# HENDRIX-ZT2/pyaudiorestoration

Measured on AMD Instinct MI355X. Metric: Msamples/sec resampled (192 kHz varispeed), higher is better.
Workload: dtype f32 near taps, far taps (|n| >= 3) as float16 hi + lo x 2^-12 filter banks on v_mfma_f32_16x16x32_f16 with f32 accumulation / f64 positions

## Files before the change

### pyaudiorestoration_amd/csrc/pos.hip

```cpp
#include "par_common.h"
#include "pos_plan.h"
#include <math.h>
#include <vector>

#pragma clang fp contract(off)

namespace par {

struct AddU128 {
  using T = U128;
  __device__ static T identity() { return T{0ull, 0ull}; }
  __device__ static T combine(T a, T b) {
    T r;
    r.lo = a.lo + b.lo;
    r.hi = a.hi + b.hi + (r.lo < a.lo ? 1ull : 0ull);
    return r;
  }
};
struct AddF64 {
  using T = double;
  __device__ static T identity() { return 0.0; }
  __device__ static T combine(T a, T b) { return a + b; }
};
struct ComposeP {
// ... 778 lines not shown
    double rr[kCk];
    const double a0 = (double)k;
#pragma unroll
    for (int u = 0; u < kCk; ++u) rr[u] = ramp_recip(a0 + (double)u, r);
#pragma unroll
    for (int u = 0; u < kCk; ++u) x = x + rr[u];
    if (k + kCk < c.n) ck[c.slot0 + k / kCk + 1] = x;
  }
  for (; k < c.k1; ++k) x = x + ramp_recip((double)k, r);
  if (__double_as_longlong(x) != __double_as_longlong(x_end)) atomicOr(&h->flags, kFlagVerify);
  if (c.j == c.J - 1) S[c.i] = x;
}

__global__ void k_inject_verify_fault(PlanHeader* __restrict__ h) { atomicOr(&h->flags, kFlagVerify); }

__global__ void k_publish_ck(PlanHeader* __restrict__ h, int64_t ck_len) {
  h->ck_len = ck_len;
  h->ck_valid = (h->flags & ~kFlagCapAmbiguous) ? 0 : 1;
  h->flags &= ~kFlagCkOverflow;
}

__device__ __forceinline__ SegFast seg_fast_record(const double* __restrict__ sp, const double* __restrict__ seg_off, long long x,
                                                   long long n) {
  const double s0 = sp[x], s1 = sp[x + 1], off = seg_off[x];
  SegFast f;
  const bool off_ok = fabs(off) < 4.0e18;
  const double ro = off_ok ? rint(off) : 0.0;
  f.foff = off_ok ? off - ro : 0.0;
  f.A = (long long)ro;
  f.n = n < 0x7fffffffll ? (int)n : 0x7fffffff;
  f.step = n >= 2 ? (s1 - s0) / (double)(n - 1) : 0.0;
  const double smin = s0 < s1 ? s0 : s1, smax = s0 < s1 ? s1 : s0;
  const double st2 = f.step * f.step, sm2 = smin * smin;
  f.fast = off_ok && n >= 2 && n < 0x7fffffffll && smin >= 0.0625 && smax <= 64.0 && st2 * st2 <= 1.296e-13 * sm2 * sm2 * smin;
  if (f.fast && fabs(f.step) <= 5.0e-5 * smin) f.fast = fabs(f.step) <= 2.7e-6 * smin ? 3 : 2;
  return f;
}

__device__ __forceinline__ void tile_entry(const double* __restrict__ sp, const int64_t* __restrict__ seg_start,
                                           const double* __restrict__ seg_off, int64_t nseg, const double* __restrict__ ck,
                                           int64_t ck_len, int64_t* __restrict__ tile_seg, long long* __restrict__ tile_st,
                                           TileHdr* __restrict__ hdr, const long long x, const long long n_tiles,
                                           const long long sample, const long long lo, const bool lazy) {
  tile_seg[x] = lo;
  for (int q = 0; q < kTileStarts; ++q) tile_st[x * kTileStarts + q] = lo + q <= nseg ? seg_start[lo + q] : LLONG_MAX;
  if (x < n_tiles) {
    const long long start = seg_start[lo], k = sample - start, b = k >> 3;
    static_assert(kCk == 8, "k >> 3");
    const double off = seg_off[lo];
    const bool off_ok = fabs(off) < 4.0e18;
    const double ro = off_ok ? rint(off) : 0.0;
    const long long slot = ck_slot0(start, lo) + b;
    const double ckv = lazy ? (lazy_segment_ok(seg_start[lo + 1] - start, sp[lo], sp[lo + 1])
                                   ? lazy_prefix(sp[lo], (sp[lo + 1] - sp[lo]) / (double)(seg_start[lo + 1] - start - 1), (double)(k + 1))
                                   : 0.0)
                            : ((b && slot < ck_len) ? ck[slot] : 0.0);
    const double rel = (off_ok ? off - ro : 0.0) + ckv;
    const bool ok = off_ok && fabs(rel) < 1.0e15 && ro > -0x1p61 && ro < 0x1p61;
    TileHdr hd;
    hd.anchor = ok ? ((long long)ro + (long long)rint(rel)) & ~1ll : 0ll;
    hd.c_last = 0;
    hd.iT = lo;
    hd.mn_rel = 0;
    bool may_unity = false, may_slow = false;
    for (long long q = lo; q < nseg && seg_start[q] <= sample + kSincTileOutputs; ++q) {
      may_unity = may_unity || !(sp[q] < kUnityHintBelow) || !(sp[q + 1] < kUnityHintBelow);
      may_slow = may_slow || !(sp[q] >= kSlowHintBelow) || !(sp[q + 1] >= kSlowHintBelow);
    }
    hd.flags = (ok ? 0 : 1) | (may_unity ? kTileMayUnity : 0) | (may_slow ? kTileMaySlow : 0) | (lazy ? kTileLazy : 0);
    hdr[x] = hd;
  }
}

__device__ __forceinline__ void tile_seg_body(const double* __restrict__ sp, const int64_t* __restrict__ seg_start,
                           const double* __restrict__ seg_off, int64_t nseg, const double* __restrict__ ck, int64_t ck_len,
                           int64_t max_tiles, int64_t* __restrict__ tile_seg, SegFast* __restrict__ seg_fast,
                           long long* __restrict__ tile_st, TileHdr* __restrict__ hdr, PlanHeader* __restrict__ h, const int64_t x) {
  const long long len_out = h->len_out;
  const long long n_tiles = (len_out + kSincTileOutputs - 1) / kSincTileOutputs;
  if (n_tiles + 1 > max_tiles) {
    if (x == 0 && len_out > 0) atomicOr(&h->flags, kFlagCkOverflow);
    return;
  }
  if (x < nseg) {
    const long long a = seg_start[x], b = seg_start[x + 1];
    if (b > a && a < len_out && ck_slot0(a, x) + (b - a + kCk - 1) / kCk > ck_len)
      atomicOr(&h->flags, kFlagCkOverflow);
    seg_fast[x] = seg_fast_record(sp, seg_off, x, b - a);
  }
  if (x > n_tiles || len_out <= 0) return;
  const long long sample = x < n_tiles ? x * kSincTileOutputs : len_out - 1;
  long long lo = 0, hi = nseg;
  while (lo < hi) {
    const long long mid = (lo + hi + 1) >> 1;
    if (seg_start[mid] <= sample) lo = mid; else hi = mid - 1;
  }
  if (lo < nseg) tile_entry(sp, seg_start, seg_off, nseg, ck, ck_len, tile_seg, tile_st, hdr, x, n_tiles, sample, lo, false);
}

__global__ void k_tile_seg(const double* __restrict__ sp, const int64_t* __restrict__ seg_start,
                           const double* __restrict__ seg_off, int64_t nseg, const double* __restrict__ ck, int64_t ck_len,
                           int64_t max_tiles, int64_t* __restrict__ tile_seg, SegFast* __restrict__ seg_fast,
                           long long* __restrict__ tile_st, TileHdr* __restrict__ hdr, PlanHeader* __restrict__ h) {
  tile_seg_body(sp, seg_start, seg_off, nseg, ck, ck_len, max_tiles, tile_seg, seg_fast, tile_st, hdr, h,
                (int64_t)blockIdx.x * blockDim.x + threadIdx.x);
}

__global__ void k_tile_seg_publish(const double* __restrict__ sp, const int64_t* __restrict__ seg_start,
                                   const double* __restrict__ seg_off, int64_t nseg, const double* __restrict__ ck, int64_t ck_len,
                                   int64_t max_tiles, int64_t* __restrict__ tile_seg, SegFast* __restrict__ seg_fast,
                                   long long* __restrict__ tile_st, TileHdr* __restrict__ hdr, PlanHeader* __restrict__ h,
                                   int64_t n_items) {
  __shared__ int is_last;
  if (h->lazy_fail) return;
  for (int64_t x0 = (int64_t)blockIdx.x * blockDim.x; x0 < n_items; x0 += (int64_t)gridDim.x * blockDim.x)
    tile_seg_body(sp, seg_start, seg_off, nseg, ck, ck_len, max_tiles, tile_seg, seg_fast, tile_st, hdr, h, x0 + threadIdx.x);
  __threadfence();
  __syncthreads();
  if (threadIdx.x == 0) is_last = atomicAdd(&h->done_tile_seg_publish, 1) == (int)gridDim.x - 1;
  __syncthreads();
  if (!is_last || threadIdx.x != 0) return;
  __threadfence();
  h->done_tile_seg_publish = 0;
  const int fl = __hip_atomic_load(&h->flags, __ATOMIC_RELAXED, __HIP_MEMORY_SCOPE_AGENT);
  h->ck_len = ck_len;
  h->ck_valid = (fl & ~kFlagCapAmbiguous) ? 0 : 1;
  h->flags = fl & ~kFlagCkOverflow;
}

__global__ __launch_bounds__(256) void k_tile_seg_lazy(const double* __restrict__ sp, const int64_t* __restrict__ seg_start,
                                                       const double* __restrict__ seg_off, int64_t nseg,
                                                       int64_t* __restrict__ tile_seg, SegFast* __restrict__ seg_fast,
                                                       long long* __restrict__ tile_st, TileHdr* __restrict__ hdr,
                                                       const PlanHeader* __restrict__ h) {
  if (h->ck_valid != 2) return;
  const long long x = (long long)blockIdx.x * blockDim.x + threadIdx.x;
  if (x >= nseg) return;
  const long long len_out = h->len_out;
  const long long n_tiles = (len_out + kSincTileOutputs - 1) / kSincTileOutputs;
  const long long a = seg_start[x], b = seg_start[x + 1];
  seg_fast[x] = seg_fast_record(sp, seg_off, x, b - a);
  if (b <= a || a >= len_out) return;
  for (long long T = (a + kSincTileOutputs - 1) / kSincTileOutputs; T * kSincTileOutputs < b && T < n_tiles; ++T)
    tile_entry(sp, seg_start, seg_off, nseg, nullptr, 0, tile_seg, tile_st, hdr, T, n_tiles, T * kSincTileOutputs, x, true);
  if (len_out - 1 < b) tile_entry(sp, seg_start, seg_off, nseg, nullptr, 0, tile_seg, tile_st, hdr, n_tiles, n_tiles, len_out - 1, x, true);
}

struct BlockPoly {
  double a0;
  double a1m1;
  double a2;
};
__device__ __forceinline__ double recip_nr(double b) {
  double x = __builtin_amdgcn_rcp(b);
  x = __builtin_fma(x, __builtin_fma(-b, x, 1.0), x);
  return __builtin_fma(x, __builtin_fma(-b, x, 1.0), x);
}
__device__ __forceinline__ BlockPoly piece_poly(double base, double rc, double z, int d0) {
  const double rp = -(rc * z), cz = rc * z * z, dd0 = (double)d0;
  const double s2m = (dd0 - 1.0) * dd0 * (2.0 * dd0 - 1.0) * (1.0 / 6.0);
  BlockPoly q;
  q.a0 = ((base + rc * (1.0 - dd0)) + 0.5 * rp * (dd0 - dd0 * dd0)) - cz * s2m;
  q.a1m1 = ((rc - 1.0) + 0.5 * rp) + cz * (1.0 / 6.0);
  q.a2 = 0.5 * rp + 0.5 * cz;
  return q;
}
__device__ __forceinline__ BlockPoly block_poly(double foff, double step, double s0, double k, int uk, double ckv, bool fast) {
  const double rc = recip_nr(__builtin_fma(step, k + 16.0, s0));
  const double z = rc * step;
  double cprev = ckv;
  if (uk) {
    if (fast) {
      const double x = z * (-0.5 * (double)(uk + 1) - 16.0);
      const double r = rc * __builtin_fma(x, __builtin_fma(x, -x, x) - 1.0, 1.0);
      cprev += r * (double)uk * __builtin_fma(z * z, (double)(uk * uk - 1) * (1.0 / 12.0), 1.0);
    } else {
      for (int v = 0; v < uk; ++v) cprev += recip_nr(__builtin_fma(step, k - (double)(uk - v), s0));
    }
  }
  return piece_poly(foff + cprev, rc, z, -16);
}
__device__ __forceinline__ bool irel_ok(long long rel) { return rel > -32000 && rel < 32000; }

__global__ __launch_bounds__(256) void k_block_rec2(const double* __restrict__ sp, const int64_t* __restrict__ seg_start,
                                                    int64_t nseg, const SegFast* __restrict__ seg_fast,
                                                    const TileHdr* __restrict__ hdr, BlockRec* __restrict__ rec,
                                                    BlockRec2* __restrict__ rec2, const PlanHeader* __restrict__ h) {
  const long long i = (long long)blockIdx.x * blockDim.x + threadIdx.x;
  if (i < 1 || i >= nseg || !h->ck_valid) return;
  const long long start = seg_start[i];
  const int us = (int)(start & (kRec - 1));
  if (us == 0 || start >= h->len_out) return;
  const SegFast s1 = seg_fast[i];
  const double rc = recip_nr(__builtin_fma(s1.step, (double)(16 - us), sp[i]));
  const BlockPoly b1 = piece_poly(s1.foff, rc, rc * s1.step, us - 16);
  const double r1 = rint(b1.a0);
  const long long rel = s1.A + (long long)r1 - hdr[start / kSincTileOutputs].anchor;
  BlockRec2 o2;
  o2.w0 = (unsigned)((int)rel << 16);
  o2.F = (float)(b1.a0 - r1);
  o2.e1 = (float)b1.a1m1;
  o2.e2 = (float)b1.a2;
  rec2[start >> kRecShift] = o2;
  if (!(fabs(b1.a0) < 1.0e9 && irel_ok(rel))) atomicOr(&rec[start >> kRecShift].w0, kRecSlow1);
}

__global__ __launch_bounds__(256) void k_block_rec(const double* __restrict__ sp, const int64_t* __restrict__ seg_start,
                                                   int64_t nseg, const double* __restrict__ ck,
                                                   const int64_t* __restrict__ tile_seg, const long long* __restrict__ tile_st,
                                                   const SegFast* __restrict__ seg_fast, const TileHdr* __restrict__ hdr,
                                                   BlockRec* __restrict__ rec, const PlanHeader* __restrict__ h) {
  const long long len_out = h->len_out;
  if (!h->ck_valid) return;
  const long long g = (long long)blockIdx.x * blockDim.x + threadIdx.x;
  const long long jb = g * kRec;
  if (jb >= len_out) return;
  const long long T = g / kBlocksPerTile;
  const long long j0 = T * kSincTileOutputs;
  const long long iT = tile_seg[T];
  int Sr[kTileStarts];
#pragma unroll
  for (int q = 0; q < kTileStarts; ++q) {
    const long long d = tile_st[T * kTileStarts + q] - j0;
    Sr[q] = d < -0x40000000ll ? -0x40000000 : (d > 0x40000000ll ? 0x40000000 : (int)d);
  }
  const int jr = (int)(jb - j0);
  int si = 0;
#pragma unroll
  for (int q = 1; q < kTileStarts; ++q) si += jr >= Sr[q];
  long long i = iT + si;
  long long k;
  double kd;
  int rem;
  long long slot0;
  if (si < kTileStarts - 1 && Sr[0] > -0x40000000) {
    int sr = Sr[0], nr = Sr[1];
#pragma unroll
    for (int q = 1; q < kTileStarts - 1; ++q) {
      if (si == q) {
        sr = Sr[q];
        nr = Sr[q + 1];
      }
    }
    k = jr - sr;
    kd = (double)(jr - sr);
    const int d = nr - jr;
    rem = d < kRec + 1 ? d : kRec + 1;
    slot0 = ck_slot0(j0 + sr, i);
  } else {
    long long hi = tile_seg[T + 1];
    while (i < hi) {
      const long long mid = (i + hi + 1) >> 1;
      if (seg_start[mid] <= jb) i = mid; else hi = mid - 1;
    }
    const long long start = seg_start[i], d = seg_start[i + 1] - jb;
    k = jb - start;
    kd = (double)k;
    rem = d < kRec + 1 ? (int)d : kRec + 1;
    slot0 = ck_slot0(start, i);
  }
  const long long i1 = i + 1 < nseg ? i + 1 : i;
  const SegFast sf = seg_fast[i];
  const SegFast s1 = seg_fast[i1];
  const double sp0 = sp[i], sp1 = sp[i1];
  const TileHdr hd = hdr[T];
  const long long b = k >> 3;
  const int uk = (int)(k & 7);
  static_assert(kCk == 8, "k >> 3");
  BlockPoly q0;
  if (hd.flags & kTileLazy) {
    const double rc = recip_nr(__builtin_fma(sf.step, kd + 16.0, sp0));
    q0 = piece_poly(sf.foff + lazy_prefix(sp0, sf.step, kd), rc, rc * sf.step, -16);
  } else {
    const double ckv = b ? ck[slot0 + b] : 0.0;
    q0 = block_poly(sf.foff, sf.step, sp0, kd, uk, ckv, sf.fast != 0);
  }
  const double r0 = rint(q0.a0);
  const long long rel0 = sf.A + (long long)(int)r0 - hd.anchor;
  const bool range0 = fabs(q0.a0) < 1.0e9 && sf.A > -(1ll << 61) && sf.A < (1ll << 61) && irel_ok(rel0) && !(hd.flags & 1);
  const unsigned ustar = rem < kRec ? (unsigned)rem : (unsigned)kRec;
  const long long ul = j0 + kSincTileOutputs >= len_out ? len_out - 1 - jb : -1;
  const unsigned slow0 = !(sf.fast >= 2 && range0 && fabs(q0.a1m1) <= 0.03125) || (ul >= 0 && ul < (long long)ustar);
  unsigned slow1 = 0u, end1 = 0u, cubic = sf.fast == 2;
  if (ustar < (unsigned)kRec) {
    const int need = kRec - (int)ustar;
    end1 = s1.n == need;
    slow1 = !(i + 1 < nseg && s1.fast >= 2 && s1.n >= need && s1.A > -(1ll << 61) && s1.A < (1ll << 61) && sp1 >= 0.971 &&
              sp1 <= 1.031) ||
            (ul >= (long long)ustar && ul < kRec);
    cubic |= s1.fast == 2;
  }
  BlockRec o;
  const bool e0 = (ustar < (unsigned)kRec) || rem == kRec;
  if (end1) slow1 = 1u;
  o.w0 = ((unsigned)((int)rel0 << 16)) | (ustar - 1u) | (e0 ? kRecE0 : 0u) | (end1 ? kRecE1 : 0u) | (slow0 ? kRecSlow0 : 0u) |
         (slow1 ? kRecSlow1 : 0u) | (cubic ? kRecCubic : 0u) | ((e0 ? ustar - 1u : 63u) << kRecLastShift);
  o.F = (float)(q0.a0 - r0);
  o.e1 = (float)q0.a1m1;
  o.e2 = (float)q0.a2;
  rec[g] = o;
}

constexpr int kRecLazySegs = 64;
#ifndef PAR_REC_EXP
#define PAR_REC_EXP 0
#endif
__device__ __forceinline__ double recip_nr_c(double b) {
#pragma clang fp contract(fast)
  double x = __builtin_amdgcn_rcp(b);
  x = x + x * (1.0 - b * x);
  return x + x * (1.0 - b * x);
}
__device__ __forceinline__ BlockPoly piece_poly_c(double base, double rc, double z, int d0) {
#pragma clang fp contract(fast)
  const double rp = -(rc * z), cz = rc * z * z, dd0 = (double)d0;
  const double s2m = (dd0 - 1.0) * dd0 * (2.0 * dd0 - 1.0) * (1.0 / 6.0);
  BlockPoly q;
  q.a0 = ((base + rc * (1.0 - dd0)) + 0.5 * rp * (dd0 - dd0 * dd0)) - cz * s2m;
  q.a1m1 = ((rc - 1.0) + 0.5 * rp) + cz * (1.0 / 6.0);
  q.a2 = 0.5 * rp + 0.5 * cz;
  return q;
}
__device__ __forceinline__ double lazy_prefix_nr(double s0, double step, double K) {
#pragma clang fp contract(fast)
  const double rc = recip_nr_c(__builtin_fma(step, 0.5 * (K - 1.0), s0));
  const double z = rc * step, t = z * z, K2 = K * K;
  return K * rc * (1.0 + t * (K2 - 1.0) * (1.0 / 12.0) * (1.0 + t * (3.0 * K2 - 7.0) * 0.05));
}
__global__ __launch_bounds__(256) void k_block_rec_lazy(const double* __restrict__ sp, const int64_t* __restrict__ seg_start,
                                                        int64_t nseg, const SegFast* __restrict__ seg_fast,
                                                        const TileHdr* __restrict__ hdr, BlockRec* __restrict__ rec,
                                                        BlockRec2* __restrict__ rec2, const PlanHeader* __restrict__ h) {
  __shared__ SegFast s_sf[4][kRecLazySegs + 1];
  __shared__ double s_sp[4][kRecLazySegs + 2];
  __shared__ int s_a[4][kRecLazySegs + 1];
  __shared__ unsigned char s_fl[4][kRecLazySegs];
  __shared__ unsigned char s_seg[4][kRecLazySegs * (kLazyMaxN / kRec)];
  static_assert(kLazyMaxN % kRec == 0 && kRecLazySegs <= 256, "a segment owns <= kLazyMaxN / kRec block starts; indices fit a byte");
  constexpr unsigned kF_Slow1 = 1u, kF_End1 = 2u, kF_Cubic1 = 4u;
  if (h->ck_valid != 2) return;
  const int l = threadIdx.x & (kWave - 1), w = threadIdx.x >> 6;
  const long long i0 = ((long long)blockIdx.x * 4 + w) * kRecLazySegs;
  if (i0 >= nseg) return;
  const long long len_out = h->len_out;
  const long long a0 = seg_start[i0];
  if (a0 >= len_out) return;
  const int nsw = (int)(nseg - i0 < kRecLazySegs ? nseg - i0 : kRecLazySegs);
  const long long G0 = (a0 + kRec - 1) >> kRecShift;
  {
    const long long il = i0 + l < nseg ? i0 + l : nseg;
    const long long al = seg_start[il];
    const long long d = al - a0;
    s_a[w][l] = d < 0x7fffffffll ? (int)d : 0x7fffffff;
    const SegFast sfl = seg_fast[il < nseg ? il : nseg - 1];
    s_sf[w][l] = sfl;
    const double spl = sp[il];
    s_sp[w][l] = spl;
    if (l == 0) {
      const long long ie = i0 + kRecLazySegs < nseg ? i0 + kRecLazySegs : nseg;
      const long long de = seg_start[ie] - a0;
      s_a[w][kRecLazySegs] = de < 0x7fffffffll ? (int)de : 0x7fffffff;
      s_sf[w][kRecLazySegs] = seg_fast[ie < nseg ? ie : nseg - 1];
      s_sp[w][kRecLazySegs] = sp[ie];
      s_sp[w][kRecLazySegs + 1] = sp[ie + 1 <= nseg ? ie + 1 : nseg];
    }
    unsigned fl = 0u;
    if (l < nsw) {
      const long long bl = seg_start[il + 1];
      const long long lim_l = bl < len_out ? bl : len_out;
      const long long g_lo = (al + kRec - 1) >> kRecShift, g_hi = (lim_l + kRec - 1) >> kRecShift;
      for (long long g = g_lo; g < g_hi; ++g) s_seg[w][g - G0] = (unsigned char)l;
      const int us = (int)(bl & (kRec - 1));
      const bool has_next = il + 1 < nseg;
      if (us != 0 && bl > al) {
        const SegFast s1 = seg_fast[has_next ? il + 1 : il];
        const double sp1 = sp[has_next ? il + 1 : il];
        const int need = kRec - us;
        if (s1.n == need) fl |= kF_End1 | kF_Slow1;
        if (!(has_next && s1.fast >= 2 && s1.n >= need && s1.A > -(1ll << 61) && s1.A < (1ll << 61) && sp1 >= 0.971 && sp1 <= 1.031))
          fl |= kF_Slow1;
        if (s1.fast == 2) fl |= kF_Cubic1;
        if (has_next && bl < len_out) {
          const long long gb = bl >> kRecShift;
          const long long anchor = hdr[(gb << kRecShift) / kSincTileOutputs].anchor;
          const double rc1 = recip_nr_c(__builtin_fma(s1.step, (double)(16 - us), sp1));
          const BlockPoly b1 = piece_poly_c(s1.foff, rc1, rc1 * s1.step, us - 16);
          const double r1 = rint(b1.a0);
          const long long rel = s1.A + (long long)r1 - anchor;
          BlockRec2 o2;
          o2.w0 = (unsigned)((int)rel << 16);
          o2.F = (float)(b1.a0 - r1);
          o2.e1 = (float)b1.a1m1;
          o2.e2 = (float)b1.a2;
          rec2[gb] = o2;
          if (!(fabs(b1.a0) < 1.0e9 && irel_ok(rel))) fl |= kF_Slow1;
        }
      }
      s_fl[w][l] = (unsigned char)fl;
    }
  }
  __builtin_amdgcn_fence(__ATOMIC_RELEASE, "wavefront");
  __builtin_amdgcn_wave_barrier();
  __builtin_amdgcn_fence(__ATOMIC_ACQUIRE, "wavefront");
  const long long b_end = a0 + s_a[w][nsw];
  const long long lim = b_end < len_out ? b_end : len_out;
  const int nblk = (int)(((lim + kRec - 1) >> kRecShift) - G0);
  const int jr0 = (int)((G0 << kRecShift) - a0);
  const long long last_tile0 = ((len_out - 1) / kSincTileOutputs) * kSincTileOutputs;
  long long Tc = -1;
  long long anchor = 0;
  int hflags = 0;
  for (int q = l; q < nblk; q += kWave) {
    const int lo = s_seg[w][q];
    const int jr = jr0 + (q << kRecShift);
    const long long g = G0 + q, jb = g << kRecShift;
    const int ar = s_a[w][lo], br = s_a[w][lo + 1];
    const SegFast sf = s_sf[w][lo];
    const double sp0 = s_sp[w][lo];
    const long long T = jb / kSincTileOutputs;
#if PAR_REC_EXP & 2
    anchor = jb;
#else
    if (T != Tc) {
      const TileHdr hd = hdr[T];
      anchor = hd.anchor;
      hflags = hd.flags;
      Tc = T;
    }
#endif
    const double kd = (double)(jr - ar);
    const int dseg = br - jr;
    const int rem = dseg < kRec + 1 ? dseg : kRec + 1;
    const double rc = recip_nr_c(__builtin_fma(sf.step, kd + 16.0, sp0));
    const BlockPoly q0 = piece_poly_c(sf.foff + lazy_prefix_nr(sp0, sf.step, kd), rc, rc * sf.step, -16);
    const double r0 = rint(q0.a0);
    const long long rel0 = sf.A + (long long)(int)r0 - anchor;
    const bool range0 = fabs(q0.a0) < 1.0e9 && sf.A > -(1ll << 61) && sf.A < (1ll << 61) && irel_ok(rel0) && !(hflags & 1);
    const unsigned ustar = rem < kRec ? (unsigned)rem : (unsigned)kRec;
    const int ul = jb >= last_tile0 ? (int)(len_out - 1 - jb) : -1;
    const unsigned slow0 = !(sf.fast >= 2 && range0 && fabs(q0.a1m1) <= 0.03125) || (ul >= 0 && ul < (int)ustar);
    unsigned slow1 = 0u, end1 = 0u, cubic = sf.fast == 2;
    if (ustar < (unsigned)kRec) {
      const unsigned fl = s_fl[w][lo];
      end1 = (fl & kF_End1) != 0u;
      slow1 = ((fl & kF_Slow1) != 0u) || (ul >= (int)ustar && ul < kRec);
      cubic |= (fl & kF_Cubic1) != 0u;
    }
    const bool e0 = (ustar < (unsigned)kRec) || rem == kRec;
    BlockRec o;
    o.w0 = ((unsigned)((int)rel0 << 16)) | (ustar - 1u) | (e0 ? kRecE0 : 0u) | (end1 ? kRecE1 : 0u) | (slow0 ? kRecSlow0 : 0u) |
           (slow1 ? kRecSlow1 : 0u) | (cubic ? kRecCubic : 0u) | ((e0 ? ustar - 1u : 63u) << kRecLastShift);
    o.F = (float)(q0.a0 - r0);
    o.e1 = (float)q0.a1m1;
    o.e2 = (float)q0.a2;
#if PAR_REC_EXP & 1
    if (o.w0 == 0x12345678u)
#endif
#if PAR_REC_EXP & 4
    {
      typedef unsigned u4v __attribute__((ext_vector_type(4)));
      u4v v = {o.w0, __float_as_uint(o.F), __float_as_uint(o.e1), __float_as_uint(o.e2)};
      __builtin_nontemporal_store(v, reinterpret_cast<u4v*>(rec + g));
    }
#else
    rec[g] = o;
#endif
  }
}

__device__ __forceinline__ void mark_direct(long long i, long long* direct, PlanHeader* h) {
  const int slot = atomicAdd(&h->n_direct, 1);
  if (slot < kMaxDirect) direct[slot] = i;
  else atomicOr(&h->flags, kFlagDirectOverflow);
}

__global__ void k_off_heads(PElem* __restrict__ el, int64_t nseg, const long long* __restrict__ direct,
                            const PlanHeader* __restrict__ h) {
  const int j = blockIdx.x * blockDim.x + threadIdx.x;
  int nd = h->n_direct;
  if (nd > kMaxDirect) nd = kMaxDirect;
  if (j == 0) el[0].head = 1;
  if (j < nd) {
    const long long d = direct[j];
    if (d + 1 < nseg) el[d + 1].head = 1;
  }
}

__device__ __forceinline__ double apply_elem(const PElem& E, double xa) {
  const int e = f64_exponent(xa);
  const long long X = (long long)ldexp(xa, 1075 - e);
  const long long Y = X + ((X & 1) ? E.c1 : E.c0);
  return ldexp((double)Y, e - 1075);
}

__global__ void k_off_stitch(const double* __restrict__ S, const PElem* __restrict__ E, const double* __restrict__ st,
                             int64_t nseg, long long* __restrict__ direct, RunEntry* __restrict__ runs,
                             PlanHeader* __restrict__ h) {
  if (threadIdx.x != 0 || blockIdx.x != 0) return;
  if (h->lazy_fail) return;
  int nd = h->n_direct;
  if (nd > kMaxDirect) nd = kMaxDirect;
  for (int a = 1; a < nd; ++a) {
    const long long v = direct[a];
    int b = a - 1;
    while (b >= 0 && direct[b] > v) {
      direct[b + 1] = direct[b];
      --b;
    }
    direct[b + 1] = v;
  }
  long long a = 0;
  double xa = st[0];
  int r = 0;
  for (int j = 0; j < nd; ++j) {
    const long long d = direct[j];
    runs[r].start = a;
    runs[r].x = xa;
    ++r;
    const double xd = (d == a) ? xa : apply_elem(E[d - 1], xa);
    xa = xd + S[d];
    a = d + 1;
  }
  runs[r].start = a;
  runs[r].x = xa;
  ++r;
  runs[r].start = INT64_MAX;
  runs[r].x = 0.0;
  h->n_direct = nd;
  h->n_runs = r;
}

__device__ __forceinline__ U128 want_fixed(const double* __restrict__ st, const double* __restrict__ sp, int64_t i, bool* bad) {
  const double period = st[i + 1] - st[i];
  const double mean = (sp[i] + sp[i + 1]) / 2.0;
  const double a = period * mean;
  U128 e{0ull, 0ull};
  if (!(a >= 0x1p-11 && a < 0x1p62)) {
    *bad = true;
  } else {
    const double ip = floor(a);
    e.hi = (unsigned long long)ip;
    e.lo = (unsigned long long)((a - ip) * 0x1p64);
  }
  return e;
}

__global__ __launch_bounds__(kScanThreads) void k_len_reduce(const double* __restrict__ st, const double* __restrict__ sp,
                                                              int64_t nseg, U128* __restrict__ bsum, double* __restrict__ partial,
                                                              PlanHeader* __restrict__ h) {
  __shared__ U128 smem[kScanThreads / kWave];
  const int64_t base = (int64_t)blockIdx.x * kScanTile + (int64_t)threadIdx.x * kScanItems;
  U128 acc = AddU128::identity();
  bool bad = false;
  double s = 0.0, c = 0.0;
#pragma unroll
  for (int k = 0; k < kScanItems; ++k) {
    if (base + k < nseg) acc = AddU128::combine(acc, want_fixed(st, sp, base + k, &bad));
    if (base + k <= nseg) {
      const double y = sp[base + k] - c;
      const double t = s + y;
      c = (t - s) - y;
      s = t;
    }
  }
  if (bad) atomicOr(&h->flags, kFlagRange);
  U128 total;
  block_exclusive<AddU128>(acc, smem, &total);
  if (threadIdx.x == 0) bsum[blockIdx.x] = total;
#pragma unroll
  for (int o = 32; o > 0; o >>= 1) s += __shfl_xor(s, o, kWave);
  if ((threadIdx.x & (kWave - 1)) == 0) partial[blockIdx.x * (kScanThreads / kWave) + threadIdx.x / kWave] = s;
}

__global__ __launch_bounds__(kScanThreads) void k_len_top(U128* __restrict__ bsum, int64_t nb, const double* __restrict__ partial,
                                                           int64_t n_part, PlanHeader* __restrict__ h) {
  __shared__ U128 smem[kScanThreads / kWave];
  __shared__ double red[kScanThreads];
  U128 carry = AddU128::identity();
  for (int64_t t0 = 0; t0 < nb; t0 += kScanTile) {
    const int64_t base = t0 + (int64_t)threadIdx.x * kScanItems;
    U128 v[kScanItems];
    U128 acc = AddU128::identity();
#pragma unroll
    for (int k = 0; k < kScanItems; ++k) {
      v[k] = (base + k < nb) ? bsum[base + k] : AddU128::identity();
      acc = AddU128::combine(acc, v[k]);
    }
    U128 total;
    U128 run = AddU128::combine(carry, block_exclusive<AddU128>(acc, smem, &total));
#pragma unroll
    for (int k = 0; k < kScanItems; ++k) {
      if (base + k < nb) bsum[base + k] = run;
      run = AddU128::combine(run, v[k]);
    }
    carry = AddU128::combine(carry, total);
  }
  double s = 0.0, c = 0.0;
  for (int64_t i = threadIdx.x; i < n_part; i += blockDim.x) {
    const double y = partial[i] - c;
    const double t = s + y;
    c = (t - s) - y;
    s = t;
  }
  red[threadIdx.x] = s;
  __syncthreads();
  for (int o = kScanThreads / 2; o > 0; o >>= 1) {
    if ((int)threadIdx.x < o) red[threadIdx.x] += red[threadIdx.x + o];
    __syncthreads();
  }
  if (threadIdx.x == 0) h->speed_sum = red[0];
}

__global__ __launch_bounds__(kScanThreads) void k_len_apply(const double* __restrict__ st, const double* __restrict__ sp,
                                                             int64_t nseg, const U128* __restrict__ bsum,
                                                             int64_t* __restrict__ seg_start, PlanHeader* __restrict__ h) {
  __shared__ U128 smem[kScanThreads / kWave];
  const int64_t base = (int64_t)blockIdx.x * kScanTile + (int64_t)threadIdx.x * kScanItems;
  U128 v[kScanItems];
  U128 acc = AddU128::identity();
  bool bad = false;
#pragma unroll
  for (int k = 0; k < kScanItems; ++k) {
    v[k] = (base + k < nseg) ? want_fixed(st, sp, base + k, &bad) : AddU128::identity();
    acc = AddU128::combine(acc, v[k]);
  }
  U128 total;
  U128 run = AddU128::combine(bsum[blockIdx.x], block_exclusive<AddU128>(acc, smem, &total));
  int f = 0;
#pragma unroll
  for (int k = 0; k < kScanItems; ++k) {
    const int64_t i = base + k;
    const U128 prev = run;
    run = AddU128::combine(run, v[k]);
    if (i >= nseg) continue;
    bool amb = false;
    const unsigned long long Ni = round_fixed(run, &amb);
    const unsigned long long Np = i > 0 ? round_fixed(prev, &amb) : 0ull;
    seg_start[i] = (int64_t)Np;
    if (i == nseg - 1) {
      seg_start[nseg] = (int64_t)Ni;
      h->total_written = (int64_t)Ni;
    }
    if (amb) f |= kFlagAmbiguous;
    if (Ni < Np + 2ull) atomicMin(&h->first_bad, (unsigned long long)i);
  }
  if (f) atomicOr(&h->flags, f);
}

__global__ __launch_bounds__(kScanThreads) void k_offs_reduce(const double* __restrict__ S, int64_t nseg, double* __restrict__ bsum) {
  __shared__ double smem[kScanThreads / kWave];
  const int64_t base = (int64_t)blockIdx.x * kScanTile + (int64_t)threadIdx.x * kScanItems;
  double acc = 0.0;
#pragma unroll
  for (int k = 0; k < kScanItems; ++k)
    if (base + k < nseg) acc = acc + S[base + k];
  double total;
  block_exclusive<AddF64>(acc, smem, &total);
  if (threadIdx.x == 0) bsum[blockIdx.x] = total;
}

__device__ __forceinline__ PElem off_element(double xa, double xb, double Si, bool* interior_out) {
  const double lo = 1.0 - 0x1p-30, hi = 1.0 + 0x1p-30;
  const int e = f64_exponent(xa);
  bool interior = xa > 0.0 && Si > 0.0 && e > 64 && e < 2046 && f64_exponent(xa * lo) == e &&
                  f64_exponent(xa * hi) == e && f64_exponent(xb * lo) == e && f64_exponent(xb * hi) == e;
  PElem p{0, 0, 0, 0};
  if (interior) {
    const double t = ldexp(Si, 1075 - e);
    if (t < 0x1p62) {
      const double fl = floor(t);
      const long long q = (long long)fl;
      const double fr = t - fl;
      if (fr > 0.5) p.c0 = p.c1 = q + 1;
      else if (fr < 0.5) p.c0 = p.c1 = q;
      else {
        p.c0 = q + (q & 1);
        p.c1 = q + ((q + 1) & 1);
      }
    } else {
      interior = false;
    }
  }
  *interior_out = interior;
  return p;
}

__global__ __launch_bounds__(kScanThreads) void k_offs_elements(const double* __restrict__ S, const double* __restrict__ st,
                                                                 int64_t nseg, const double* __restrict__ bsum_f,
                                                                 PElem* __restrict__ el, long long* __restrict__ direct,
                                                                 PlanHeader* __restrict__ h, Cand* __restrict__ cand,
                                                                 const double* __restrict__ sp,
                                                                 const int64_t* __restrict__ seg_start) {
  __shared__ double smem_f[kScanThreads / kWave];
  const int64_t base = (int64_t)blockIdx.x * kScanTile + (int64_t)threadIdx.x * kScanItems;
  double v[kScanItems];
  double acc = 0.0;
#pragma unroll
  for (int k = 0; k < kScanItems; ++k) {
    v[k] = (base + k < nseg) ? S[base + k] : 0.0;
    acc = acc + v[k];
  }
  double total;
  double run = bsum_f[blockIdx.x] + block_exclusive<AddF64>(acc, smem_f, &total);
  const double st0 = st[0];
#pragma unroll
  for (int k = 0; k < kScanItems; ++k) {
    const int64_t i = base + k;
    const double xa = st0 + run;
    run = run + v[k];
    if (i >= nseg) continue;
    bool interior;
    PElem p = off_element(xa, st0 + run, v[k], &interior);
    if (!interior) mark_direct(i, direct, h);
    el[i] = p;
    if (cand != nullptr) {
      bool listed = !interior;
      if (interior) {
        const int e = f64_exponent(xa);
        const double t = ldexp(v[k], 1075 - e);
        const double fr = t - floor(t);
        const double dist = fabs(fr - 0.5);
        if (!(dist > ldexp(lazy_bound((double)kLazyMaxN, 0.0625), 1075 - e))) {
          const double s0 = sp[i], s1 = sp[i + 1];
          const double bu = ldexp(lazy_bound((double)(seg_start[i + 1] - seg_start[i]), s0 < s1 ? s0 : s1), 1075 - e);
          listed = !(dist > bu);
        }
      }
      if (listed) {
        const int slot = atomicAdd(&h->n_cand, 1);
        if (slot < kMaxCand) cand[slot] = Cand{(long long)i, xa, st0 + run};
      }
    }
  }
}


__global__ __launch_bounds__(256) void k_seg_sum_lazy(const double* __restrict__ sp, const int64_t* __restrict__ seg_start,
                                                      int64_t nseg, double* __restrict__ S, PlanHeader* __restrict__ h) {
  const int64_t i = (int64_t)blockIdx.x * blockDim.x + threadIdx.x;
  if (i >= nseg) return;
  const long long n = seg_start[i + 1] - seg_start[i];
  const double s0 = sp[i], s1 = sp[i + 1];
  double v = 0.0;
  if (lazy_segment_ok(n, s0, s1)) {
    v = lazy_prefix(s0, (s1 - s0) / (double)(n - 1), (double)n);
  } else {
    atomicOr(&h->lazy_fail, 1);
  }
  S[i] = v;
}

__global__ __launch_bounds__(64) void k_seg_exact_list(const double* __restrict__ sp, const int64_t* __restrict__ seg_start,
                                                       int64_t nseg, double* __restrict__ S, PElem* __restrict__ el,
                                                       const Cand* __restrict__ cand, long long* __restrict__ direct,
                                                       PlanHeader* __restrict__ h) {
  const int slot = blockIdx.x * blockDim.x + threadIdx.x;
  int nc = h->n_cand;
  if (nc > kMaxCand) {
    if (slot == 0) atomicOr(&h->lazy_fail, 2);
    return;
  }
  if (slot >= nc || h->lazy_fail) return;
  const Cand c = cand[slot];
  const long long i = c.i;
  const long long n = seg_start[i + 1] - seg_start[i];
  const Ramp r = make_ramp(sp[i], sp[i + 1], n);
  double sum = 0.0;
  long long k = 0;
  for (; k + 8 <= n; k += 8) {
// ... 647 lines not shown
```

Before: 196,700.

## Stage per-segment reciprocals and tile anchors in LDS for lazy block-record kernel

Restructures k_block_rec_lazy so each lane precomputes the segment reciprocal, its scaled step and a relative anchor offset into LDS. Tile headers covering the wave's range are staged once in LDS instead of being reloaded from global memory per tile. The per-block fast path replaces the double Newton reciprocal and prefix series with a cheaper polynomial series expansion in 32-bit relative arithmetic, and a wave-uniform fallback keeps the old exact path for saturated or out-of-range cases. The aim is fewer f64 divides and global loads per block record, at the cost of extra LDS, a second wave barrier and accuracy that depends on the series truncation.

Result: no change. 197,400 (median of 6 runs) (+0.3%).

```diff
diff --git a/pyaudiorestoration_amd/csrc/pos.hip b/pyaudiorestoration_amd/csrc/pos.hip
--- a/pyaudiorestoration_amd/csrc/pos.hip
+++ b/pyaudiorestoration_amd/csrc/pos.hip
@@ -1104,9 +1104,14 @@
 }
 
 constexpr int kRecLazySegs = 64;
-#ifndef PAR_REC_EXP
-#define PAR_REC_EXP 0
-#endif
+constexpr int kRecLazyTiles = kRecLazySegs * (int)(kLazyMaxN / kSincTileOutputs) + 2;
+constexpr int kTileShift = 10;
+static_assert(kSincTileOutputs == 1 << kTileShift && kLazyMaxN <= kSincTileOutputs && kBlocksPerTile == 1 << (kTileShift - kRecShift),
+              "a block's tile by shifts; 64 segments of <= kLazyMaxN outputs from anywhere in a tile touch <= 66 tiles");
+__device__ __forceinline__ double recip_1p(double e) {
+  const double e2 = e * e, a = 1.0 - e;
+  return __builtin_fma(__builtin_fma(e2, e2, e2), a, a);
+}
 __device__ __forceinline__ double recip_nr_c(double b) {
 #pragma clang fp contract(fast)
   double x = __builtin_amdgcn_rcp(b);
@@ -1129,144 +1134,184 @@
   const double z = rc * step, t = z * z, K2 = K * K;
   return K * rc * (1.0 + t * (K2 - 1.0) * (1.0 / 12.0) * (1.0 + t * (3.0 * K2 - 7.0) * 0.05));
 }
+__device__ __forceinline__ double lazy_prefix_ser(double r0, double eta, double em, double K) {
+#pragma clang fp contract(fast)
+  const double g = recip_1p(em);
+  const double rc = r0 * g, z = eta * g, zK = z * K, w = zK * zK;
+  return (K * rc) * (1.0 + (w - z * z) * (1.0 + 0.15 * w) * (1.0 / 12.0));
+}
 __global__ __launch_bounds__(256) void k_block_rec_lazy(const double* __restrict__ sp, const int64_t* __restrict__ seg_start,
                                                         int64_t nseg, const SegFast* __restrict__ seg_fast,
                                                         const TileHdr* __restrict__ hdr, BlockRec* __restrict__ rec,
                                                         BlockRec2* __restrict__ rec2, const PlanHeader* __restrict__ h) {
-  __shared__ SegFast s_sf[4][kRecLazySegs + 1];
-  __shared__ double s_sp[4][kRecLazySegs + 2];
-  __shared__ int s_a[4][kRecLazySegs + 1];
-  __shared__ unsigned char s_fl[4][kRecLazySegs];
+  struct Staged {
+    double foff, r0, eta;
+    int a;
+    int rel;
+    unsigned fl;
+    int pad;
+  };
+  __shared__ Staged s_sg[4][kRecLazySegs + 1];
+  __shared__ int s_tile[4][kRecLazyTiles];
   __shared__ unsigned char s_seg[4][kRecLazySegs * (kLazyMaxN / kRec)];
   static_assert(kLazyMaxN % kRec == 0 && kRecLazySegs <= 256, "a segment owns <= kLazyMaxN / kRec block starts; indices fit a byte");
-  constexpr unsigned kF_Slow1 = 1u, kF_End1 = 2u, kF_Cubic1 = 4u;
-  if (h->ck_valid != 2) return;
-  const int l = threadIdx.x & (kWave - 1), w = threadIdx.x >> 6;
+  constexpr unsigned kF_Ok0 = 1u;
+  constexpr unsigned kF_Old = 2u;
+  constexpr int kT_Range = 1, kT_Sat = 2;
+  static_assert(kF_Ok0 == (unsigned)kT_Range, "one bit test for the segment's and the tile's verdict");
+  static_assert(kRecLazyTiles <= 2 * kWave, "a lane stages at most two tile headers");
+  const int l = threadIdx.x & (kWave - 1);
+  const int w = __builtin_amdgcn_readfirstlane((int)(threadIdx.x >> 6));
   const long long i0 = ((long long)blockIdx.x * 4 + w) * kRecLazySegs;
   if (i0 >= nseg) return;
+  const int nsw = (int)(nseg - i0 < kRecLazySegs ? nseg - i0 : kRecLazySegs);
+  const int ck_valid = h->ck_valid;
   const long long len_out = h->len_out;
   const long long a0 = seg_start[i0];
-  if (a0 >= len_out) return;
-  const int nsw = (int)(nseg - i0 < kRecLazySegs ? nseg - i0 : kRecLazySegs);
+  const long long b_end = seg_start[i0 + nsw];
+  const unsigned long long Aref = (unsigned long long)seg_fast[i0].A;
+  if (ck_valid != 2 || a0 >= len_out) return;
   const long long G0 = (a0 + kRec - 1) >> kRecShift;
+  const long long lim = b_end < len_out ? b_end : len_out;
+  const int nblk = (int)(((lim + kRec - 1) >> kRecShift) - G0);
+  const long long T0 = a0 >> kTileShift;
+  const TileHdr* __restrict__ hdrT = hdr + T0;
+  const int off0 = (int)((G0 << kRecShift) - (T0 << kTileShift));
+  const int ntile = nblk > 0 ? ((off0 + ((nblk - 1) << kRecShift)) >> kTileShift) + 1 : 1;
+  const long long il = i0 + l < nseg ? i0 + l : nseg;
+  const long long al = seg_start[il];
+  const long long bl = seg_start[l < nsw ? il + 1 : il];
+  const SegFast sfl = seg_fast[il < nseg ? il : nseg - 1];
+  const double spl = sp[il];
   {
-    const long long il = i0 + l < nseg ? i0 + l : nseg;
-    const long long al = seg_start[il];
-    const long long d = al - a0;
-    s_a[w][l] = d < 0x7fffffffll ? (int)d : 0x7fffffff;
-    const SegFast sfl = seg_fast[il < nseg ? il : nseg - 1];
-    s_sf[w][l] = sfl;
-    const double spl = sp[il];
-    s_sp[w][l] = spl;
-    if (l == 0) {
-      const long long ie = i0 + kRecLazySegs < nseg ? i0 + kRecLazySegs : nseg;
-      const long long de = seg_start[ie] - a0;
-      s_a[w][kRecLazySegs] = de < 0x7fffffffll ? (int)de : 0x7fffffff;
-      s_sf[w][kRecLazySegs] = seg_fast[ie < nseg ? ie : nseg - 1];
-      s_sp[w][kRecLazySegs] = sp[ie];
-      s_sp[w][kRecLazySegs + 1] = sp[ie + 1 <= nseg ? ie + 1 : nseg];
-    }
-    unsigned fl = 0u;
-    if (l < nsw) {
-      const long long bl = seg_start[il + 1];
-      const long long lim_l = bl < len_out ? bl : len_out;
-      const long long g_lo = (al + kRec - 1) >> kRecShift, g_hi = (lim_l + kRec - 1) >> kRecShift;
-      for (long long g = g_lo; g < g_hi; ++g) s_seg[w][g - G0] = (unsigned char)l;
-      const int us = (int)(bl & (kRec - 1));
-      const bool has_next = il + 1 < nseg;
-      if (us != 0 && bl > al) {
-        const SegFast s1 = seg_fast[has_next ? il + 1 : il];
-        const double sp1 = sp[has_next ? il + 1 : il];
-        const int need = kRec - us;
-        if (s1.n == need) fl |= kF_End1 | kF_Slow1;
-        if (!(has_next && s1.fast >= 2 && s1.n >= need && s1.A > -(1ll << 61) && s1.A < (1ll << 61) && sp1 >= 0.971 && sp1 <= 1.031))
-          fl |= kF_Slow1;
-        if (s1.fast == 2) fl |= kF_Cubic1;
-        if (has_next && bl < len_out) {
-          const long long gb = bl >> kRecShift;
-          const long long anchor = hdr[(gb << kRecShift) / kSincTileOutputs].anchor;
-          const double rc1 = recip_nr_c(__builtin_fma(s1.step, (double)(16 - us), sp1));
-          const BlockPoly b1 = piece_poly_c(s1.foff, rc1, rc1 * s1.step, us - 16);
-          const double r1 = rint(b1.a0);
-          const long long rel = s1.A + (long long)r1 - anchor;
-          BlockRec2 o2;
-          o2.w0 = (unsigned)((int)rel << 16);
-          o2.F = (float)(b1.a0 - r1);
-          o2.e1 = (float)b1.a1m1;
-          o2.e2 = (float)b1.a2;
-          rec2[gb] = o2;
-          if (!(fabs(b1.a0) < 1.0e9 && irel_ok(rel))) fl |= kF_Slow1;
-        }
+    long long an[2] = {0, 0};
+    int tf[2] = {0, 0};
+#pragma unroll
+    for (int k = 0; k < 2; ++k) {
+      if (l + k * kWave < ntile) {
+        an[k] = hdrT[l + k * kWave].anchor;
+        tf[k] = hdrT[l + k * kWave].flags;
       }
-      s_fl[w][l] = (unsigned char)fl;
-    }
-  }
+    }
+#pragma unroll
+    for (int k = 0; k < 2; ++k) {
+      if (l + k * kWave < ntile) {
+        const unsigned long long d = (unsigned long long)an[k] - Aref;
+        s_tile[w][l + k * kWave] = (int)((unsigned)d << 2) | (d + (1ull << 29) < (1ull << 30) ? 0 : kT_Sat) | (tf[k] & kT_Range);
+      }
+    }
+  }
+  const long long d = al - a0;
+  s_sg[w][l].a = d < 0x7fffffffll ? (int)d : 0x7fffffff;
+  const double r0l = recip_nr_c(spl);
+  s_sg[w][l].foff = sfl.foff;
+  s_sg[w][l].r0 = r0l;
+  s_sg[w][l].eta = sfl.step * r0l;
+  const unsigned long long dA = (unsigned long long)sfl.A - Aref;
+  s_sg[w][l].rel = (int)(unsigned)dA;
+  if (l == 0) {
+    const long long de = b_end - a0;
+    s_sg[w][kRecLazySegs].a = de < 0x7fffffffll ? (int)de : 0x7fffffff;
+  }
+  const unsigned own = (sfl.fast >= 2 && sfl.A > -(1ll << 61) && sfl.A < (1ll << 61) ? kF_Ok0 : 0u) | (sfl.fast == 2 ? kRecCubic : 0u) |
+                       (sfl.n >= kRec && dA + (1ull << 29) < (1ull << 30) ? 0u : kF_Old);
   __builtin_amdgcn_fence(__ATOMIC_RELEASE, "wavefront");
   __builtin_amdgcn_wave_barrier();
   __builtin_amdgcn_fence(__ATOMIC_ACQUIRE, "wavefront");
-  const long long b_end = a0 + s_a[w][nsw];
-  const long long lim = b_end < len_out ? b_end : len_out;
-  const int nblk = (int)(((lim + kRec - 1) >> kRecShift) - G0);
+  if (l < nsw) {
+    unsigned fl = 0u;
+    const long long lim_l = bl < len_out ? bl : len_out;
+    const long long g_lo = (al + kRec - 1) >> kRecShift, g_hi = (lim_l + kRec - 1) >> kRecShift;
+    for (long long g = g_lo; g < g_hi; ++g) s_seg[w][g - G0] = (unsigned char)l;
+    const int us = (int)(bl & (kRec - 1));
+    const bool has_next = il + 1 < nseg;
+    if (us != 0 && bl > al) {
+      const SegFast s1 = seg_fast[has_next ? il + 1 : il];
+      const double sp1 = sp[has_next ? il + 1 : il];
+      const int need = kRec - us;
+      if (s1.n == need) fl |= kRecE1 | kRecSlow1;
+      if (!(has_next && s1.fast >= 2 && s1.n >= need && s1.A > -(1ll << 61) && s1.A < (1ll << 61) && sp1 >= 0.971 && sp1 <= 1.031))
+        fl |= kRecSlow1;
+      if (s1.fast == 2) fl |= kRecCubic;
+      if (has_next && bl < len_out) {
+        const long long gb = bl >> kRecShift;
+        const int dt2 = (int)(((gb << kRecShift) - (T0 << kTileShift)) >> kTileShift);
+        const int tw2 = s_tile[w][dt2];
+        const double rc1 = recip_nr_c(__builtin_fma(s1.step, (double)(16 - us), sp1));
+        const BlockPoly b1 = piece_poly_c(s1.foff, rc1, rc1 * s1.step, us - 16);
+        const double r1 = rint(b1.a0);
+        const long long rel = (tw2 & kT_Sat) ? s1.A + (long long)r1 - hdrT[dt2].anchor
+                                             : (long long)((unsigned long long)s1.A - Aref) + (long long)r1 - (long long)(tw2 >> 2);
+        BlockRec2 o2;
+        o2.w0 = (unsigned)((int)rel << 16);
+        o2.F = (float)(b1.a0 - r1);
+        o2.e1 = (float)b1.a1m1;
+        o2.e2 = (float)b1.a2;
+        rec2[gb] = o2;
+        if (!(fabs(b1.a0) < 1.0e9 && irel_ok(rel))) fl |= kRecSlow1;
+      }
+    }
+    s_sg[w][l].fl = fl | (own << 16);
+  }
+  __builtin_amdgcn_fence(__ATOMIC_RELEASE, "wavefront");
+  __builtin_amdgcn_wave_barrier();
+  __builtin_amdgcn_fence(__ATOMIC_ACQUIRE, "wavefront");
   const int jr0 = (int)((G0 << kRecShift) - a0);
-  const long long last_tile0 = ((len_out - 1) / kSincTileOutputs) * kSincTileOutputs;
-  long long Tc = -1;
-  long long anchor = 0;
-  int hflags = 0;
+  const long long dlast = len_out - 1 - (G0 << kRecShift);
+  const int qlast = dlast < 0x40000000ll ? (int)dlast : 0x40000000;
+  BlockRec* __restrict__ recW = rec + G0;
   for (int q = l; q < nblk; q += kWave) {
     const int lo = s_seg[w][q];
-    const int jr = jr0 + (q << kRecShift);
-    const long long g = G0 + q, jb = g << kRecShift;
-    const int ar = s_a[w][lo], br = s_a[w][lo + 1];
-    const SegFast sf = s_sf[w][lo];
-    const double sp0 = s_sp[w][lo];
-    const long long T = jb / kSincTileOutputs;
-#if PAR_REC_EXP & 2
-    anchor = jb;
-#else
-    if (T != Tc) {
-      const TileHdr hd = hdr[T];
-      anchor = hd.anchor;
-      hflags = hd.flags;
-      Tc = T;
-    }
-#endif
-    const double kd = (double)(jr - ar);
+    const int qo = q << kRecShift;
+    const int jr = jr0 + qo;
+    const Staged* sg = &s_sg[w][lo];
+    const int ar = sg[0].a, br = sg[1].a;
+    const unsigned fl = sg->fl, own = fl >> 16;
+    const int dt = (off0 + qo) >> kTileShift;
+    const int tw = s_tile[w][dt];
+    const double foff = sg->foff;
     const int dseg = br - jr;
-    const int rem = dseg < kRec + 1 ? dseg : kRec + 1;
-    const double rc = recip_nr_c(__builtin_fma(sf.step, kd + 16.0, sp0));
-    const BlockPoly q0 = piece_poly_c(sf.foff + lazy_prefix_nr(sp0, sf.step, kd), rc, rc * sf.step, -16);
-    const double r0 = rint(q0.a0);
-    const long long rel0 = sf.A + (long long)(int)r0 - anchor;
-    const bool range0 = fabs(q0.a0) < 1.0e9 && sf.A > -(1ll << 61) && sf.A < (1ll << 61) && irel_ok(rel0) && !(hflags & 1);
-    const unsigned ustar = rem < kRec ? (unsigned)rem : (unsigned)kRec;
-    const int ul = jb >= last_tile0 ? (int)(len_out - 1 - jb) : -1;
-    const unsigned slow0 = !(sf.fast >= 2 && range0 && fabs(q0.a1m1) <= 0.03125) || (ul >= 0 && ul < (int)ustar);
-    unsigned slow1 = 0u, end1 = 0u, cubic = sf.fast == 2;
-    if (ustar < (unsigned)kRec) {
-      const unsigned fl = s_fl[w][lo];
-      end1 = (fl & kF_End1) != 0u;
-      slow1 = ((fl & kF_Slow1) != 0u) || (ul >= (int)ustar && ul < kRec);
-      cubic |= (fl & kF_Cubic1) != 0u;
-    }
-    const bool e0 = (ustar < (unsigned)kRec) || rem == kRec;
+    BlockPoly q0;
+    double r0;
+    int rel0;
+    bool irel0;
+    if (__ballot((own & kF_Old) != 0u || (tw & kT_Sat) != 0) == 0ull) {
+#pragma clang fp contract(fast)
+      const double sr0 = sg->r0, eta = sg->eta;
+      const double k17 = (double)(jr - ar + 17);
+      const double ec = __builtin_fma(eta, k17, -eta);
+      const double g = recip_1p(ec);
+      const double rc = sr0 * g, z = eta * g, rz = rc * z, cz = rz * z;
+      q0.a0 = foff + lazy_prefix_ser(sr0, eta, 0.5 * ec, k17);
+      q0.a1m1 = ((rc - 1.0) - 0.5 * rz) + cz * (1.0 / 6.0);
+      q0.a2 = 0.5 * cz - 0.5 * rz;
+      r0 = rint(q0.a0);
+      rel0 = sg->rel + (int)r0 - (tw >> 2);
+      irel0 = rel0 > -32000 && rel0 < 32000;
+    } else {
+      const SegFast sf = seg_fast[i0 + lo];
+      const double sp0 = sp[i0 + lo], kd = (double)(jr - ar);
+      const double rc = recip_nr_c(__builtin_fma(sf.step, kd + 16.0, sp0));
+      q0 = piece_poly_c(foff + lazy_prefix_nr(sp0, sf.step, kd), rc, rc * sf.step, -16);
+      r0 = rint(q0.a0);
+      const long long rel = sf.A + (long long)(int)r0 - hdrT[dt].anchor;
+      rel0 = (int)rel;
+      irel0 = irel_ok(rel);
+    }
+    const unsigned um1 = (unsigned)(dseg < kRec ? dseg : kRec) - 1u;
+    const bool good = (own & ~(unsigned)tw & kF_Ok0) != 0u && fabs(q0.a0) < 1.0e9 && irel0 && fabs(q0.a1m1) <= 0.03125;
+    unsigned bits = (own & kRecCubic) | (dseg < kRec ? fl & (kRecE1 | kRecSlow1 | kRecCubic) : 0u) | (good ? 0u : kRecSlow0);
+    const unsigned ul = (unsigned)(qlast - qo);
+    if (__ballot(ul < (unsigned)kRec) != 0ull) {
+      if (ul < (unsigned)kRec) bits |= ul <= um1 ? kRecSlow0 : kRecSlow1;
+    }
+    const unsigned lastu = dseg <= kRec ? kRecE0 | (um1 << kRecLastShift) : 63u << kRecLastShift;
     BlockRec o;
-    o.w0 = ((unsigned)((int)rel0 << 16)) | (ustar - 1u) | (e0 ? kRecE0 : 0u) | (end1 ? kRecE1 : 0u) | (slow0 ? kRecSlow0 : 0u) |
-           (slow1 ? kRecSlow1 : 0u) | (cubic ? kRecCubic : 0u) | ((e0 ? ustar - 1u : 63u) << kRecLastShift);
+    o.w0 = ((unsigned)rel0 << 16) | um1 | lastu | bits;
     o.F = (float)(q0.a0 - r0);
     o.e1 = (float)q0.a1m1;
     o.e2 = (float)q0.a2;
-#if PAR_REC_EXP & 1
-    if (o.w0 == 0x12345678u)
-#endif
-#if PAR_REC_EXP & 4
-    {
-      typedef unsigned u4v __attribute__((ext_vector_type(4)));
-      u4v v = {o.w0, __float_as_uint(o.F), __float_as_uint(o.e1), __float_as_uint(o.e2)};
-      __builtin_nontemporal_store(v, reinterpret_cast<u4v*>(rec + g));
-    }
-#else
-    rec[g] = o;
-#endif
+    recW[(unsigned)q] = o;
   }
 }
 
```
